# M4THYOU/TokenDagger

Hardware: AMD Instinct MI355X
Metric: GB/s raw text tokenized (Llama-4 vocab, 1024 MB corpus) (higher is better)
Workload: dtype u8; 1 GPU; Llama-4-Scout vocab, 1024 MiB synthetic english text, 1741775 documents, CoreBPE::encode semantics, input resident in HBM; bytes=1073741824, docs=1741775, bytes_rank0=1073741824, docs_rank0=1741775, parallelism=single GPU

## Files before the change

### tokendagger_amd/csrc/td_common.h

```cpp
#pragma once
#include <stdint.h>

#include "../../include/tokendagger_hip.h"

#if defined(__HIP__)
#define TD_HD __host__ __device__ inline __attribute__((always_inline))
#else
#define TD_HD inline
#endif

namespace td {

enum : uint32_t {
    C_OTHER = 0,
    C_APOS = 1,
    C_SLASH = 2,
    C_SP = 3,
    C_WS = 4,
    C_CRLF = 5,
    C_UP = 6,
    C_LW = 7,
    C_LB = 8,
    C_MK = 9,
    C_NUM = 10,
// ... 501 lines not shown
    MK_COUNT
};
struct BitWin {
    uint64_t m[MK_COUNT];
};

TD_HD int td_ctz64(uint64_t x) {
#if defined(__HIP_DEVICE_COMPILE__)
    return x ? (int)__builtin_ctzll(x) : 64;
#else
    return x ? (int)__builtin_ctzll(x) : 64;
#endif
}
TD_HD int td_top64(uint64_t x) { return 64 - (int)__builtin_clzll(x); }
TD_HD int td_run_end(uint64_t m, int f) { return f >= 64 ? 64 : f + td_ctz64(~(m >> f)); }
TD_HD uint64_t td_bits_below(int n) { return n >= 64 ? ~0ull : ((1ull << n) - 1ull); }

TD_HD uint32_t mask_bits_of(uint32_t vp, uint32_t v, uint32_t pv = 0) {
    const uint32_t c = v & CLS_MASK;
    uint32_t r = 0;
    r |= in_set(M_U, c) ? (1u << MK_U) : 0u;
    r |= in_set(M_W, c) ? (1u << MK_W) : 0u;
    r |= in_set(M_X, c) ? (1u << MK_X) : 0u;
    r |= in_set(M_S, c) ? (1u << MK_S) : 0u;
    r |= (c == C_NUM) ? (1u << MK_N) : 0u;
    r |= (c == C_CRLF) ? (1u << MK_CR) : 0u;
    r |= in_set(M_TRAIL, c) ? (1u << MK_TR) : 0u;
    r |= (v & F_CONT) ? (1u << MK_C) : 0u;
    r |= (v & F_DOC) ? (1u << MK_D) : 0u;
    r |= (c == C_APOS) ? (1u << MK_A) : 0u;
    r |= (c == C_SP) ? (1u << MK_SP) : 0u;
    r |= is_sync(vp, v, pv) ? (1u << MK_SYNC) : 0u;
    return r;
}
struct WinP {
    const BitWin& w;
    int o, lim;
    uint64_t E;
    TD_HD WinP(const BitWin& w_, int o_, int avail) : w(w_), o(o_), lim(avail), E(w_.m[MK_D] & ~td_bits_below(o_ + 1)) {}
    TD_HD bool bit(int k, int i) const { return (w.m[k] >> i) & 1ull; }
    TD_HD bool ebit(int i) const { return (E >> i) & 1ull; }
    TD_HD int run_end(int k, int from) const { return td_run_end(w.m[k] & ~E, from); }
    TD_HD int run_end2(int k1, int k2, int from) const { return td_run_end((w.m[k1] | w.m[k2]) & ~E, from); }
    TD_HD int last_and(int k1, int k2, int lo, int hi) const {
        const uint64_t m = w.m[k1] & w.m[k2] & td_bits_below(hi) & ~td_bits_below(lo);
        return m ? td_top64(m) - 1 : -1;
    }
    TD_HD int last_set(int k, int lo, int hi) const {
        const uint64_t m = w.m[k] & td_bits_below(hi) & ~td_bits_below(lo);
        return m ? td_top64(m) - 1 : -1;
    }
    TD_HD int last_clear(int k, int lo, int hi) const {
        const uint64_t m = ~w.m[k] & td_bits_below(hi) & ~td_bits_below(lo);
        return m ? td_top64(m) - 1 : -1;
    }
};

struct BitWin32 {
    uint32_t m[MK_COUNT];
};
TD_HD int td_ctz32(uint32_t x) { return x ? (int)__builtin_ctz(x) : 32; }
struct WinP32 {
    const BitWin32& w;
    int o, lim;
    uint32_t E;
    TD_HD WinP32(const BitWin32& w_, int avail) : w(w_), o(0), lim(avail), E(w_.m[MK_D] & ~1u) {}
    TD_HD bool bit(int k, int i) const { return (w.m[k] >> i) & 1u; }
    TD_HD bool ebit(int i) const { return (E >> i) & 1u; }
    TD_HD int run_end(int k, int from) const { return from >= 32 ? 32 : from + td_ctz32(~((w.m[k] & ~E) >> from)); }
    TD_HD int run_end2(int k1, int k2, int from) const {
        return from >= 32 ? 32 : from + td_ctz32(~(((w.m[k1] | w.m[k2]) & ~E) >> from));
    }
    TD_HD static uint32_t below(int n) { return n >= 32 ? ~0u : ((1u << n) - 1u); }
    TD_HD int last_and(int k1, int k2, int lo, int hi) const {
        const uint32_t m = w.m[k1] & w.m[k2] & below(hi) & ~below(lo);
        return m ? 31 - (int)__builtin_clz(m) : -1;
    }
    TD_HD int last_set(int k, int lo, int hi) const {
        const uint32_t m = w.m[k] & below(hi) & ~below(lo);
        return m ? 31 - (int)__builtin_clz(m) : -1;
    }
    TD_HD int last_clear(int k, int lo, int hi) const {
        const uint32_t m = ~w.m[k] & below(hi) & ~below(lo);
        return m ? 31 - (int)__builtin_clz(m) : -1;
    }
};

template <class B>
TD_HD int scan_piece_fast32(const BitWin32& v, int avail, const B& bytes, uint32_t pv) {
    if (pv & (PV_GPT2 | PV_LEADING_CONTRACTION | PV_PLAIN_LETTERS | PV_WS_EOS_FIRST)) return -1;
    const uint32_t U = v.m[MK_U], W = v.m[MK_W], X = v.m[MK_X], S = v.m[MK_S], N = v.m[MK_N], CR = v.m[MK_CR], TR = v.m[MK_TR];
    const uint32_t C = v.m[MK_C], A = v.m[MK_A], SP = v.m[MK_SP];
    const uint32_t E = v.m[MK_D] & ~1u;
    const uint32_t lim = avail >= 32 ? 0u : ~0u << avail;
    const uint32_t Ue = U & ~E, We = W & ~E, Xe = X & ~E, Se = S & ~E, TRe = TR & ~E;
    const int p1 = 1 + td_ctz32(~(C >> 1));
    const bool u0 = U & 1u, w0 = W & 1u, x0 = X & 1u, s0 = S & 1u, n0 = N & 1u, cr0 = CR & 1u;
    bool bad = p1 >= avail || p1 > 4;
    const int p1c = p1 > 31 ? 31 : p1;
    const bool l0 = u0 || w0;
    const bool l1 = (x0 || s0) && !((E >> p1c) & 1u) && (((U | W) >> p1c) & 1u);
    const bool letters = !cr0 && !n0 && (l0 || l1);
    bad = bad || (letters && l0 && l1);
    const int st = l1 ? p1c : 0;
    const int q = st + td_ctz32(~(Ue >> st));
    const int qc = q > 31 ? 31 : q;
    const bool wf = ((We >> qc) & 1u) && q < 32;
    const int ew = wf ? qc + td_ctz32(~(We >> qc)) : q;
    const uint32_t uw = U & W & ((qc == 0 ? 0u : (~0u >> (32 - qc)))) & (~0u << st);
    const int e1 = wf ? ew : (uw ? 32 - (int)__builtin_clz(uw) : 0);
    const int el = e1 ? e1 : (q > st ? ew : 0);
    int e_let = el;
    if (!(pv & PV_NO_CONTRACTION)) {
        const int ec = el > 29 ? 29 : el;
        const bool apo = ((A >> ec) & 1u) && !((v.m[MK_D] >> ec) & 1u) && !((v.m[MK_D] >> (ec + 1)) & 1u);
        if (letters && el > 0 && apo) {
            if (el + 3 > avail) bad = true;
            else {
                const uint32_t b1 = bytes(el + 1), b2 = bytes(el + 2);
                const bool d2 = (v.m[MK_D] >> (ec + 2)) & 1u;
                const uint32_t c1 = b1 | 0x20u, c2 = b2 | 0x20u;
                if (b1 < 0x80u && (c1 == 's' || c1 == 't' || c1 == 'm' || c1 == 'd')) e_let = el + 2;
                else if (b1 < 0x80u && !d2 && b2 < 0x80u && ((c1 == 'r' && c2 == 'e') || (c1 == 'v' && c2 == 'e') || (c1 == 'l' && c2 == 'l'))) e_let = el + 3;
                else if (b1 == 0xC5u && !d2 && b2 == 0xBFu) e_let = el + 3;
            }
        }
    }
    bad = bad || (letters && (el == 0 || q >= avail || ew >= avail || el + 3 > avail));
    const int nmax = (pv & PV_SINGLE_DIGIT) ? 1 : 3;
    const int nrun = td_ctz32(~(N & ~E) | (1u << nmax));
    const int e_num = nrun < 1 ? 1 : nrun;
    bad = bad || (n0 && ((C & 0xEu) || e_num + 1 > avail));
    const bool psp = (SP & 1u) && ((X >> 1) & 1u) && !((E >> 1) & 1u);
    const bool punct = psp || x0;
    const int pst = psp ? 1 : 0;
    const int px = pst + td_ctz32(~(Xe >> pst));
    const int pxc = px > 31 ? 31 : px;
    const int e_p = px >= 32 ? 32 : pxc + td_ctz32(~(TRe >> pxc));
    bad = bad || (!letters && !n0 && punct && (px >= avail || e_p >= avail));
    const int sq = td_ctz32(~Se);
    const uint32_t below = sq >= 32 ? ~0u : ((1u << sq) - 1u);
    const uint32_t crs = CR & below;
    const uint32_t leads = ~C & below & ~1u;
    const int e_s = crs ? 32 - (int)__builtin_clz(crs)
                        : (sq < 32 && ((E >> sq) & 1u)) ? sq
                        : leads ? 31 - (int)__builtin_clz(leads) : sq;
    bad = bad || (!letters && !n0 && !punct && s0 && sq >= avail);
    (void)lim;
    const int e = letters ? e_let : n0 ? e_num : punct ? e_p : s0 ? e_s : p1;
    return (bad || e <= 0 || e > avail) ? -1 : e;
}

TD_HD uint64_t td_land(uint64_t M, uint64_t A) { return ((M + (A & M)) & ~M) | (A & ~M); }
TD_HD uint64_t td_brev64(uint64_t x) {
#if defined(__clang__)
    return __builtin_bitreverse64(x);
#else
    x = ((x >> 1) & 0x5555555555555555ull) | ((x & 0x5555555555555555ull) << 1);
    x = ((x >> 2) & 0x3333333333333333ull) | ((x & 0x3333333333333333ull) << 2);
    x = ((x >> 4) & 0x0F0F0F0F0F0F0F0Full) | ((x & 0x0F0F0F0F0F0F0F0Full) << 4);
    return __builtin_bswap64(x);
#endif
}
constexpr uint32_t PV_WORD_RULES_OK = PV_NO_CONTRACTION | PV_SINGLE_DIGIT;
TD_HD uint64_t split_unresolved_heads(const BitWin& w, uint32_t pv, uint64_t* extra = nullptr) {
    const uint64_t SY = w.m[MK_SYNC];
    if (extra) *extra = 0;
    if (pv & ~PV_WORD_RULES_OK) return SY;
    const uint64_t nD = ~w.m[MK_D];
    const uint64_t U = w.m[MK_U] & nD, W = w.m[MK_W] & nD, X = w.m[MK_X] & nD, S = w.m[MK_S] & nD, N = w.m[MK_N] & nD;
    const uint64_t CR = w.m[MK_CR] & nD, TR = w.m[MK_TR] & nD, C = w.m[MK_C] & nD, SP = w.m[MK_SP] & nD;
    const uint64_t H = SY & nD;
    const uint64_t L = U | W, Up = U & ~W, Xn = X & ~L;
    const uint64_t pfx = H & (X | S) & ~CR & ~L;
    const uint64_t p1 = td_land(C, pfx << 1);
    const uint64_t a1 = (H & L) | (p1 & L);
    uint64_t good = td_land(W, td_land(Up, a1));
    const uint64_t hn = H & N;
    const uint64_t near = (pv & PV_SINGLE_DIGIT) ? (hn << 1) : ((hn << 1) | (hn << 2) | (hn << 3));
    const uint64_t ln = td_land(N, hn);
    good |= ln & near;
    if (extra && hn && !(pv & PV_SINGLE_DIGIT)) {
        const uint64_t NC = N & ~C;
        const uint64_t e3 = (hn << 3) & NC & (NC << 1) & (NC << 2);
        good |= ln & ((e3 << 1) | (e3 << 2) | (e3 << 3));
        *extra = e3;
    }
    const uint64_t b1 = (H & Xn) | ((H & SP & (Xn >> 1)) << 1);
    good |= td_land(TR, td_land(Xn, b1));
    const uint64_t hs = H & S;
    good |= td_land(S, hs) & ((CR << 1) | (hs << 1));
    const uint64_t bad_end = SY & ~good;
    const uint64_t zr = td_brev64(~SY);
    const uint64_t start = (td_brev64(bad_end) << 1) | 1ull;
    return td_brev64(td_land(zr, start));
}

struct ArrMaskP {
    const uint64_t* arr;
    int o, lim;
    TD_HD ArrMaskP(const uint64_t* a, int o_, int lim_) : arr(a), o(o_), lim(lim_) {}
    TD_HD uint64_t word(int k, int wi) const { return arr[wi * MK_COUNT + k]; }
    TD_HD uint64_t eword(int wi) const {
        const int wo = o >> 6;
        if (wi < wo) return 0;
        const uint64_t d = word(MK_D, wi);
        return wi == wo ? d & ~td_bits_below((o & 63) + 1) : d;
    }
    TD_HD bool bit(int k, int i) const { return (word(k, i >> 6) >> (i & 63)) & 1ull; }
    TD_HD bool ebit(int i) const { return i > o && bit(MK_D, i); }
    TD_HD int run_end(int k, int from) const {
        int i = from;
        while (i < lim) {
            const int wi = i >> 6, sh = i & 63;
            const uint64_t m = (word(k, wi) & ~eword(wi)) >> sh;
            const int t = td_ctz64(~m);
            if (t < 64 - sh) return i + t;
            i += 64 - sh;
        }
        return i;
    }
    TD_HD int run_end2(int k1, int k2, int from) const {
        int i = from;
        while (i < lim) {
            const int wi = i >> 6, sh = i & 63;
            const uint64_t m = ((word(k1, wi) | word(k2, wi)) & ~eword(wi)) >> sh;
            const int t = td_ctz64(~m);
            if (t < 64 - sh) return i + t;
            i += 64 - sh;
        }
        return i;
    }
    template <class F>
    TD_HD int last_where(const F& f, int lo, int hi) const {
        if (hi <= lo) return -1;
        for (int wi = (hi - 1) >> 6; wi >= (lo >> 6); --wi) {
            uint64_t m = f(wi);
            const int base = wi << 6;
            if (hi - base < 64) m &= td_bits_below(hi - base);
            if (lo > base) m &= ~td_bits_below(lo - base);
            if (m) return base + td_top64(m) - 1;
        }
        return -1;
    }
    TD_HD int last_and(int k1, int k2, int lo, int hi) const {
        return last_where([&](int wi) { return word(k1, wi) & word(k2, wi); }, lo, hi);
    }
    TD_HD int last_set(int k, int lo, int hi) const {
        return last_where([&](int wi) { return word(k, wi); }, lo, hi);
    }
    TD_HD int last_clear(int k, int lo, int hi) const {
        return last_where([&](int wi) { return ~word(k, wi); }, lo, hi);
    }
};

enum : int { CM_U = 0, CM_W, CM_X, CM_S, CM_NRAW, CM_CR, CM_TR, CM_C, CM_SYNC, CM_COUNT };
template <class V, class W>
TD_HD void cm_expand(V& v, const W* s, W d) {
    v.m[MK_U] = s[CM_U]; v.m[MK_W] = s[CM_W]; v.m[MK_X] = s[CM_X]; v.m[MK_S] = s[CM_S];
    v.m[MK_N] = s[CM_NRAW] & ~(s[CM_X] | s[CM_S]);
    v.m[MK_CR] = s[CM_CR]; v.m[MK_TR] = s[CM_TR]; v.m[MK_C] = s[CM_C];
    v.m[MK_D] = d;
    v.m[MK_A] = s[CM_NRAW] & s[CM_X];
    v.m[MK_SP] = s[CM_NRAW] & s[CM_S];
    v.m[MK_SYNC] = s[CM_SYNC];
}
struct CompactMaskP {
    const uint32_t* arr;
    const uint32_t* doc;
    int stride;
    int o, lim;
    TD_HD CompactMaskP(const uint32_t* a, int stride_, const uint32_t* d, int o_, int lim_) : arr(a), doc(d), stride(stride_), o(o_), lim(lim_) {}
    TD_HD uint64_t stored(int s, int wi) const { return ((uint64_t)arr[s * stride + 2 * wi + 1] << 32) | arr[s * stride + 2 * wi]; }
    TD_HD uint64_t dword64(int wi) const { return ((uint64_t)doc[2 * wi + 1] << 32) | doc[2 * wi]; }
    TD_HD uint64_t word(int k, int wi) const {
        switch (k) {
            case MK_U: return stored(CM_U, wi);
            case MK_W: return stored(CM_W, wi);
            case MK_X: return stored(CM_X, wi);
            case MK_S: return stored(CM_S, wi);
            case MK_N: return stored(CM_NRAW, wi) & ~(stored(CM_X, wi) | stored(CM_S, wi));
            case MK_CR: return stored(CM_CR, wi);
            case MK_TR: return stored(CM_TR, wi);
            case MK_C: return stored(CM_C, wi);
            case MK_D: return dword64(wi);
            case MK_A: return stored(CM_NRAW, wi) & stored(CM_X, wi);
            case MK_SP: return stored(CM_NRAW, wi) & stored(CM_S, wi);
            default: return stored(CM_SYNC, wi);
        }
    }
    TD_HD uint64_t eword(int wi) const {
        const int wo = o >> 6;
        if (wi < wo) return 0;
        const uint64_t d = dword64(wi);
        return wi == wo ? d & ~td_bits_below((o & 63) + 1) : d;
    }
    TD_HD bool bit(int k, int i) const { return (word(k, i >> 6) >> (i & 63)) & 1ull; }
    TD_HD bool ebit(int i) const { return i > o && bit(MK_D, i); }
    template <class F>
    TD_HD int run_where(const F& f, int from) const {
        int i = from;
        while (i < lim) {
            const int wi = i >> 6, sh = i & 63;
            const uint64_t m = (f(wi) & ~eword(wi)) >> sh;
            const int t = td_ctz64(~m);
            if (t < 64 - sh) return i + t;
            i += 64 - sh;
        }
        return i;
    }
    TD_HD int run_end(int k, int from) const { return run_where([&](int wi) { return word(k, wi); }, from); }
    TD_HD int run_end2(int k1, int k2, int from) const { return run_where([&](int wi) { return word(k1, wi) | word(k2, wi); }, from); }
    template <class F>
    TD_HD int last_where(const F& f, int lo, int hi) const {
        if (hi <= lo) return -1;
        for (int wi = (hi - 1) >> 6; wi >= (lo >> 6); --wi) {
            uint64_t m = f(wi);
            const int base = wi << 6;
            if (hi - base < 64) m &= td_bits_below(hi - base);
            if (lo > base) m &= ~td_bits_below(lo - base);
            if (m) return base + td_top64(m) - 1;
        }
        return -1;
    }
    TD_HD int last_and(int k1, int k2, int lo, int hi) const { return last_where([&](int wi) { return word(k1, wi) & word(k2, wi); }, lo, hi); }
    TD_HD int last_set(int k, int lo, int hi) const { return last_where([&](int wi) { return word(k, wi); }, lo, hi); }
    TD_HD int last_clear(int k, int lo, int hi) const { return last_where([&](int wi) { return ~word(k, wi); }, lo, hi); }
};

template <class P, class B>
TD_HD int scan_contraction_p(const P& p, const B& bytes, int e, bool leading = false) {
    if (e + 3 > p.lim) return -1;
    if (!p.bit(MK_A, e) || (p.bit(MK_D, e) && !leading)) return e;
    if (p.bit(MK_D, e + 1)) return e;
    const uint32_t b1 = bytes(e + 1);
    const bool d2 = p.bit(MK_D, e + 2);
    if (b1 < 0x80) {
        const uint32_t l1 = b1 | 0x20;
        if (l1 == 's' || l1 == 't' || l1 == 'm' || l1 == 'd') return e + 2;
        if (d2) return e;
        const uint32_t b2 = bytes(e + 2);
        if (b2 < 0x80) {
            const uint32_t l2 = b2 | 0x20;
            if ((l1 == 'r' && l2 == 'e') || (l1 == 'v' && l2 == 'e') || (l1 == 'l' && l2 == 'l')) return e + 3;
// ... 322 lines not shown
```

### tokendagger_amd/csrc/td_kernels.hip

```cpp
#include <hip/hip_runtime.h>
#include <stdlib.h>

#include "td_kernels.h"

namespace td {

#ifdef TD_ABLATE
#define TD_STOP(n) (a.stop_after == (n))
#else
#define TD_STOP(n) false
#endif

struct LdsSrc {
    const uint8_t* txt;
    const uint32_t* docw;
    int64_t lo, hi;
    __device__ __forceinline__ uint32_t byte(int64_t i) const { return txt[i]; }
    __device__ __forceinline__ bool doc(int64_t i) const { return (docw[i >> 5] >> (i & 31)) & 1u; }
};
struct GlobSrc {
    const uint8_t* text;
    const uint32_t* docbits;
    int64_t lo, hi;
    __device__ __forceinline__ uint32_t byte(int64_t i) const { return text[i]; }
// ... 1026 lines not shown
                auto bytes_below = [](int nb) { return nb >= 8 ? ~0ull : ((1ull << (8 * nb)) - 1ull); };
                {
                    const int lc0 = td_ctz64(~ct & HB) >> 3, lcd = (int)td_ctz32(docb | 0x100u);
                    lead_conts = lc0 < lcd ? lc0 : lcd;
                }
                uint32_t kj[4], ndj[4], cpj[4], uj[4];
                bool tbj[4];
#pragma unroll
                for (int j = 0; j < 4; ++j) {
                    const bool have = ld != 0;
                    const int k = have ? td_ctz64(ld) >> 3 : 0;
                    ld &= ld - 1ull;
#ifndef TD_DECODE_BRANCHY
                    const uint32_t dlo = k < 4 ? t8.x : t8.y, dhi = k < 4 ? t8.y : t8n.x;
                    const uint32_t x = __funnelshift_r(dlo, dhi, 8u * ((uint32_t)k & 3u));
                    const uint32_t b = x & 0xFFu;
                    const uint32_t need = utf8_declared_len(b) - 1u;
                    const int pos = pos0 + k;
                    const uint32_t cm = (0xC0C0C000u >> (8u * (3u - need))) & 0xC0C0C000u;
                    const bool ok = have & (need > 0) & (pos + (int)need < (int)src.hi) & (pos >= (int)src.lo) & (((docb >> (k + 1)) & ((1u << need) - 1u)) == 0u) &
                                    ((x & cm) == (cm & 0x80808000u));
                    const uint32_t c1 = (x >> 8) & 0x3Fu, c2 = (x >> 16) & 0x3Fu, c3 = (x >> 24) & 0x3Fu;
                    uint32_t c = ((b & (0x3Fu >> need)) << 6) | c1;
                    c = need >= 2u ? (c << 6) | c2 : c;
                    c = need >= 3u ? (c << 6) | c3 : c;
#else
                    const uint64_t hi8 = ((uint64_t)t8n.y << 32) | t8n.x;
                    const uint64_t w = (lo8 >> (8 * k)) | ((hi8 << 8) << (56 - 8 * k));
                    const uint32_t b = (uint32_t)w & 0xFFu, c1 = (uint32_t)(w >> 8) & 0xFFu, c2 = (uint32_t)(w >> 16) & 0xFFu, c3 = (uint32_t)(w >> 24) & 0xFFu;
                    const uint32_t need = utf8_declared_len(b) - 1u;
                    const int pos = pos0 + k;
                    const bool ok = have && need > 0 && pos + (int)need < (int)src.hi && pos >= (int)src.lo && !((docb >> (k + 1)) & ((1u << need) - 1u)) &&
                                    (c1 & 0xC0) == 0x80 && (need < 2 || (c2 & 0xC0) == 0x80) && (need < 3 || (c3 & 0xC0) == 0x80);
                    const uint32_t c = (need == 1) ? ((b & 0x1F) << 6) | (c1 & 0x3F)
                                     : (need == 2) ? ((b & 0x0F) << 12) | ((c1 & 0x3F) << 6) | (c2 & 0x3F)
                                                   : ((b & 0x07) << 18) | ((c1 & 0x3F) << 12) | ((c2 & 0x3F) << 6) | (c3 & 0x3F);
#endif
                    tbj[j] = ok && c <= 0x10FFFFu && !(c >= 0xD800u && c <= 0xDFFFu);
                    cpj[j] = tbj[j] ? c : 0u;
                    kj[j] = (uint32_t)k;
                    ndj[j] = ok ? need : 0u;
                    uj[j] = t_u1[cpj[j] >> 8];
                }
#pragma unroll
                for (int j = 0; j < 4; ++j) uj[j] = t_u2[uj[j] * 256u + (cpj[j] & 255u)];
                uint64_t cov = 0;
                int remaining = 0, last_lead = -1;
#pragma unroll
                for (int j = 0; j < 4; ++j) {
                    if (ndj[j]) {
                        const uint32_t f = tbj[j] ? (uint32_t)s_fcls[uj[j] & 15u] : (uint32_t)FB_X;
                        const uint32_t bm = ndj[j] == 3u ? 0xFFFFFFFFu : ((1u << (8u * (ndj[j] + 1u))) - 1u);
                        const uint32_t pat = ((f * 0x01010101u) | 0x80808000u) & bm;
                        const int sh = 8 * (int)kj[j];
                        F = (F & ~((uint64_t)bm << sh)) | ((uint64_t)pat << sh);
                        cov |= (uint64_t)(bm & 0x80808080u) << sh;
                        last_lead = (int)kj[j];
                        remaining = ((int)kj[j] + (int)ndj[j] > 7) ? (int)kj[j] + (int)ndj[j] - 7 : 0;
                    }
                }
                const uint64_t lcm = bytes_below(lead_conts);
                for (uint64_t gen = na & ~cov & ~lcm; gen; gen &= gen - 1ull) {
                    const int k = td_ctz64(gen) >> 3;
                    const uint32_t f = feature_at_v(t_ascii, t_u1, t_u2, s_txt, s_doc, (int)src.lo, (int)src.hi, pos0 + k);
                    F = (F & ~(0xFFull << (8 * k))) | ((uint64_t)f << (8 * k));
                }
                F &= ~lcm;
                flo = (uint32_t)F;
                fhi = (uint32_t)(F >> 32);
                const uint64_t starts = HB & ~(cov & ct) & ~lcm;
                if (starts) {
                    const int last = (63 - (int)__builtin_clzll(starts)) >> 3;
                    st_out = ((uint32_t)(F >> (8 * last)) & 0x7Fu) | ((uint32_t)(last == last_lead ? remaining : 0) << 9);
                } else {
                    st_out = 0x100u;
                }
            }
            {
                uint32_t st_in = __shfl_up(st_out, 1);
                if (lane == 0) st_in = carry_st;
                carry_st = (uint32_t)__builtin_amdgcn_readlane((int)st_out, 63);
                if (lead_conts) {
                    const bool known = !(st_in & 0x100u);
                    const int claim = (int)(st_in >> 9);
                    for (int k = 0; k < lead_conts; ++k) {
                        const uint32_t f = (known && k < claim) ? ((st_in & 0xFFu) | FB_C) : feature_at_v(t_ascii, t_u1, t_u2, s_txt, s_doc, (int)src.lo, (int)src.hi, it * 8 + k);
                        if (k < 4) flo |= f << (8 * k); else fhi |= f << (8 * (k - 4));
                    }
                }
            }
            uint32_t pf = __shfl_up(fhi >> 24, 1);
            if (lane == 0 && q > 0) pf = carry_pf;
            carry_pf = (uint32_t)__builtin_amdgcn_readlane((int)(fhi >> 24), 63);
            if (lane == 0 && q == 0) {
                pf = 0;
                if (it > 0) {
                    const uint32_t pb = s_txt[it * 8 - 1];
                    pf = (pb < 0x80) ? (uint32_t)s_lut[pb] : feature_at_v(t_ascii, t_u1, t_u2, s_txt, s_doc, (int)src.lo, (int)src.hi, it * 8 - 1);
                }
            }
            emit_masks(it, flo, fhi, pf);
        }
        }
        __syncthreads();
        FZ_TICK(1)
        if (tid == 0) s_nonascii = 0;
        if (TD_STOP(12)) continue;

        {
            constexpr bool FAST = !(PV & (PV_GPT2 | PV_LEADING_CONTRACTION | PV_PLAIN_LETTERS | PV_WS_EOS_FIRST));
            auto load_view64 = [&](BitWin& v, int j) {
                uint64_t s[CM_COUNT];
#pragma unroll
                for (int k = 0; k < CM_COUNT; ++k) s[k] = ((uint64_t)s_cm[k * CM_STRIDE + j + 1] << 32) | s_cm[k * CM_STRIDE + j];
                cm_expand(v, s, ((uint64_t)s_doc[j + 1] << 32) | s_doc[j]);
            };
            auto load_view32 = [&](BitWin32& v, int j, uint32_t sh) {
                uint32_t s[CM_COUNT];
#pragma unroll
                for (int k = 0; k < CM_COUNT; ++k) s[k] = __funnelshift_r(s_cm[k * CM_STRIDE + j], s_cm[k * CM_STRIDE + j + 1], sh);
                cm_expand(v, s, __funnelshift_r(s_doc[j], s_doc[j + 1], sh));
            };
            auto defer = [&](int64_t g) {
                if (FUSED) s_defer = 1;
                const uint32_t q = atomicAdd(a->slow_count, 1u);
                if (q < a->slow_cap) a->slow_list[q] = g;
                else raise(a, TD_E_SCRATCH, g);
            };
            auto mark = [&](int q) { atomicOr(&s_start[q >> 5], 1u << (q & 31)); };
            auto sync_at = [&](int q) { return (s_cm[CM_SYNC * CM_STRIDE + (q >> 5)] >> (q & 31)) & 1u; };
            auto crossed = [&](int e) {
                if (FUSED) s_cross = e;
                if (tile + 1 < a->n_stiles) a->tile_carry[tile + 1] = wg0 + e;
            };
            auto walk = [&](int p) {
                for (;;) {
                    const int e = scan_piece_lds<PV>(s_cm, s_doc, s_txt, p);
                    if (e < 0) { if (p >= K_HL) defer(wg0 + p); return; }
                    if (e >= tile_hi) { crossed(e); return; }
                    if (sync_at(e)) return;
                    if (e >= K_HL) mark(e);
                    p = e;
                }
            };
            const int b0 = K_HL + tid * 32;
            uint32_t mine = 0;
            uint32_t extra_hi = 0;
            {
                BitWin wv;
                load_view64(wv, b0 >> 5);
                uint32_t sy = (uint32_t)wv.m[MK_SYNC];
                const int room = tile_hi - b0;
                if (room < 32) sy = room <= 0 ? 0u : sy & ((1u << room) - 1u);
                uint32_t st0 = sy, un;
                if (wv.m[MK_N] != 0ull) {
                    uint64_t extra = 0;
                    un = (uint32_t)split_unresolved_heads(wv, PV, &extra) & sy;
                    extra &= (uint64_t)sy << 3;
                    extra &= room >= 64 ? ~0ull : room <= 0 ? 0ull : ((1ull << room) - 1ull);
                    st0 |= (uint32_t)extra;
                    extra_hi = (uint32_t)(extra >> 32);
                } else {
                    un = (uint32_t)split_unresolved_heads(wv, PV) & sy;
                }
                s_start[b0 >> 5] = st0;
                if (sy) atomicMax(&s_last, b0 + 31 - (int)__clz(sy));
                const uint32_t cnt = __popc(un);
                const uint32_t incl = wave_incl_scan(cnt, lane);
                uint32_t base = 0;
                if (lane == 63 && incl) base = atomicAdd(&s_nh, incl);
                base = (uint32_t)__builtin_amdgcn_readlane((int)base, 63);
                uint32_t idx = base + incl - cnt;
                while (un) {
                    const int bit = __ffs(un) - 1;
                    un &= un - 1u;
                    if (idx < (uint32_t)KS_HCAP) s_heads[idx] = (uint16_t)(b0 + bit); else mine |= 1u << bit;
                    ++idx;
                }
            }
            __syncthreads();
            FZ_TICK(2)
            if (extra_hi) atomicOr(&s_start[(b0 >> 5) + 1], extra_hi);
            if (TD_STOP(13)) continue;
            {
                const uint32_t nh = s_nh < (uint32_t)KS_HCAP ? s_nh : (uint32_t)KS_HCAP;
                int p = -1;
                if (tid == 0) {
                    static_assert(K_HL % 64 == 0 && K_HL >= 64, "left halo = whole mask words");
                    const uint32_t* const sync32 = s_cm + CM_SYNC * CM_STRIDE;
                    if (!(sync32[K_HL / 32] & 1u)) {
                        int sp = -1;
                        for (int w = K_HL / 64 - 1; w >= 0 && sp < 0; --w) {
                            uint64_t m = ((uint64_t)sync32[2 * w + 1] << 32) | sync32[2 * w];
                            if (w == 0) m &= ~0xFull;
                            if (m) sp = w * 64 + td_top64(m) - 1;
                        }
                        if (sp < 0) { a->tile_flag[tile] = 1; atomicAdd(a->far_count, 1u); if (FUSED) s_defer = 1; }
                        else p = sp;
                    }
                }
                if (tid == 1 && s_last >= 0) p = s_last;
                bool more = true;
                for (;;) {
                    const uint64_t nb = __ballot(p < 0);
                    if (nb && more) {
                        uint32_t base = 0;
                        if (lane == __ffsll((unsigned long long)nb) - 1) base = atomicAdd(&s_cur, (uint32_t)__popcll(nb));
                        base = (uint32_t)__builtin_amdgcn_readlane((int)base, __ffsll((unsigned long long)nb) - 1);
                        more = base + (uint32_t)__popcll(nb) < nh;
                        if (p < 0) {
                            const uint32_t idx = base + __builtin_amdgcn_mbcnt_hi((uint32_t)(nb >> 32), __builtin_amdgcn_mbcnt_lo((uint32_t)nb, 0u));
                            if (idx < nh) p = s_heads[idx];
                        }
                    }
                    if (!__ballot(p >= 0)) break;
                    if (p >= 0) {
                        BitWin32 v;
                        load_view32(v, p >> 5, (uint32_t)(p & 31));
                        const int avail = (K_LIM - p < 32) ? (K_LIM - p) : 32;
                        auto bytes = [&](int q) { return (uint32_t)s_txt[p + q]; };
                        const int r = FAST ? scan_piece_fast32(v, avail, bytes, PV) : scan_piece_p(WinP32(v, avail), bytes, PV);
                        if (r < 0) {
                            const uint32_t ci = atomicAdd(&s_ncold, 1u);
                            if (ci < (uint32_t)KS_CCAP) s_cold[ci] = (uint16_t)p; else walk(p);
                            p = -1;
                        } else {
                            const int e = p + r;
                            bool stop = true;
                            if (e >= tile_hi) crossed(e);
                            else {
                                stop = (r < 32) ? ((v.m[MK_SYNC] >> r) & 1u) : sync_at(e);
                                if (!stop && e >= K_HL) mark(e);
                            }
                            p = stop ? -1 : e;
                        }
                    }
                }
            }
            __syncthreads();
            {
                const uint32_t nc = s_ncold < (uint32_t)KS_CCAP ? s_ncold : (uint32_t)KS_CCAP;
                for (uint32_t i = tid; i < nc; i += K_THREADS) walk(s_cold[i]);
                while (mine) {
                    const int bit = __ffs(mine) - 1;
                    mine &= mine - 1u;
                    walk(b0 + bit);
                }
            }
        }
        __syncthreads();
        FZ_TICK(3)
        if (tid < KS_TILE / 32) {
            const int64_t g = tile_g0 + (int64_t)tid * 32;
            if (g < a->n) {
                uint32_t v = s_start[K_HL / 32 + tid];
                if (g + 32 > a->n) v &= (1u << (int)(a->n - g)) - 1u;
                TD_NT_STORE(v, &a->startbits[(tile_g0 >> 5) + tid]);
            }
        }
        if constexpr (DRAW) {
            if constexpr (!DIRECT) {
                next_tile = __builtin_amdgcn_readfirstlane(s_next[par]);
                if (tid == 0) s_next[par ^ 1] = (int)(2u * gridDim.x + atomicAdd(a->tile_draw, 1u));
                par = __builtin_amdgcn_readfirstlane(par ^ 1);
            } else {
                next_tile = __builtin_amdgcn_readfirstlane(s_next[0]);
            }
            if (next_tile < a->n_stiles) load_window((int64_t)next_tile * KS_TILE - K_HL);
        } else if (FUSED && tile + (int)gridDim.x < a->n_stiles) {
            load_window(wg0 + (int64_t)gridDim.x * KS_TILE);
        }
        }
        if constexpr (FUSED) {
            constexpr int NT4 = KS_TILE / K_TILE;
            static_assert(NT4 == 2 && KS_CHUNK == 32, "two token tiles, a 32-bit START word per lane");
            const int cross = s_cross;
            const bool tile_deferred = s_defer != 0 || cross < 0;
            uint16_t* const s_plist = reinterpret_cast<uint16_t*>(s_R + FZ_R_PLIST);
            uint16_t* const s_coldk = reinterpret_cast<uint16_t*>(s_R + FZ_R_COLDK);
            uint16_t* const s_pb = reinterpret_cast<uint16_t*>(s_R + FZ_R_PB);
            const int wv = tid >> 6;
            const int tile4 = tile * NT4;
            const bool two = K_HL + K_TILE < tile_hi;
            const int b0 = K_HL + tid * KS_CHUNK;
            const uint32_t smask0 = s_start[b0 >> 5];
            const uint32_t cnt = __popc(smask0);
            const uint32_t incl = wave_incl_scan(cnt, lane);
            if (lane == 63) s_wave[wv] = incl;
            if (tid == 0) { s_hflags[0] = 0; s_hflags[1] = 0; s_nrec[0] = 0; s_nrec[1] = 0; s_ncoldp = 0; }
            __syncthreads();
            const uint32_t w0s = s_wave[0], w1s = s_wave[1], w2s = s_wave[2], w3s = s_wave[3];
            const uint32_t np = w0s + w1s + w2s + w3s, n0 = w0s + w1s;
            const uint32_t pbase = (wv > 0 ? w0s : 0u) + (wv > 1 ? w1s : 0u) + (wv > 2 ? w2s : 0u) + incl - cnt;
            const bool cand = DIRECT && !s_brk;
            auto break_chain = [&]() {
                __hip_atomic_store(&a->tile_state[tile], TS_BROKEN << 62, __ATOMIC_RELAXED, __HIP_MEMORY_SCOPE_AGENT);
                s_brk = 1u;
            };
            if (tile_deferred || np > (uint32_t)FZ_NPC) {
                if (tid == 0) {
                    const uint32_t at = atomicAdd(a->deferred_count, two ? 2u : 1u);
                    a->deferred_list[at] = (uint32_t)tile4;
                    if (two) a->deferred_list[at + 1] = (uint32_t)tile4 + 1u;
                    if (DIRECT) break_chain();
                }
            } else {
                {
                    uint32_t k = pbase, m = smask0;
                    while (m) {
                        const int b = __ffs(m) - 1;
                        m &= m - 1;
                        s_plist[k++] = (uint16_t)(b0 + b);
                    }
                }
                s_pb[tid] = (uint16_t)pbase;
                if (tid == 0) s_plist[np] = (uint16_t)cross;
                const uint64_t fdd = fd0 != 0xFFFFFFFFu ? fd0 : fd1;
                if (cand && tid == 0) { s_pd[ring][PD_FDD] = (uint32_t)fdd; s_pd[ring][PD_TILE] = (uint32_t)tile; s_pd[ring][PD_NP] = np; s_pd[ring][PD_N0] = n0; }
                const int64_t dmine = (int64_t)fdd + tid;
                const int64_t dpos = (fdd != 0xFFFFFFFFu && dmine < a->n_docs) ? a->doc_offsets[dmine] : a->n;
                __syncthreads();
                FZ_TICK(4)
                uint32_t* const slab = a->slab + ((size_t)blockIdx.x * SLAB_RING + ring) * SLAB_WORDS;
                uint32_t* const dst0 = cand ? slab : a->stage + (size_t)tile4 * K_STAGE;
                uint32_t* const dst1 = cand ? slab : dst0 + K_STAGE - n0;
                auto note_miss = [&](uint32_t k, uint32_t res) {
                    const uint32_t h = k >= n0 ? 1u : 0u;
                    const uint32_t mi = atomicAdd(&s_nrec[h], 1u);
                    if (mi < (uint32_t)K_MISS_LISTED_MAX) s_rec[h][mi] = ((k - (h ? n0 : 0u)) << 19) | (res & 0x7FFFFu);
                };
                auto miss_marker = [&](int i, uint32_t len) { return TOK_MISS | ((uint32_t)((i - K_HL) & (K_TILE - 1)) << 7) | len; };
                typedef uint32_t u32x4 __attribute__((ext_vector_type(4)));
                typedef const u32x4 __attribute__((address_space(1)))* gslot_t;
                gslot_t const p12 = (gslot_t)(uintptr_t)T->piece12_slots;
                const uint32_t p12_mask = T->piece12_mask;
                const bool fastpath = a->use_fastpath != 0;
                for (uint32_t kb = tid; kb < np; kb += K_THREADS * FZ_PB) {
                    u32x4 sl[FZ_PB];
                    uint32_t kk0[FZ_PB], kk1[FZ_PB], kk2[FZ_PB], il[FZ_PB];
#pragma unroll
                    for (int q = 0; q < FZ_PB; ++q) {
                        const uint32_t k = kb + (uint32_t)q * K_THREADS;
                        const bool on = k < np;
                        const int i = on ? s_plist[k] : K_HL;
                        const uint32_t len = on ? (uint32_t)s_plist[k + 1] - (uint32_t)i : 0u;
                        const uint32_t* wp = reinterpret_cast<const uint32_t*>(s_txt) + (i >> 2);
                        const uint32_t sh = (i & 3) * 8;
                        const uint32_t w0 = wp[0], w1 = wp[1], w2 = wp[2], w3 = wp[3];
                        const uint4 km = reinterpret_cast<const uint4*>(s_kmask)[len < P12_MAXLEN ? len : P12_MAXLEN];
                        kk0[q] = __funnelshift_r(w0, w1, sh) & km.x;
                        kk1[q] = __funnelshift_r(w1, w2, sh) & km.y;
                        kk2[q] = __funnelshift_r(w2, w3, sh) & km.z;
                        il[q] = ((uint32_t)i << 16) | (len < 0xFFFFu ? len : 0xFFFFu);
                        if (on) sl[q] = p12[hash_piece12(kk0[q], kk1[q], kk2[q], len) & p12_mask];
                    }
#pragma unroll
                    for (int q = 0; q < FZ_PB; ++q) {
                        const uint32_t k = kb + (uint32_t)q * K_THREADS;
                        if (k < np) {
                            const int i = (int)(il[q] >> 16);
                            const uint32_t len = il[q] & 0xFFFFu;
                            const u32x4 e = sl[q];
                            if (len <= P12_MAXLEN && fastpath &&
                                (e.w == 0u || (e.x == kk0[q] && e.y == kk1[q] && e.z == kk2[q] && (e.w >> 24) == (0x80u | len)))) {
                                const bool miss = e.w == 0u;
                                const uint32_t res = miss ? miss_marker(i, len) : (e.w & 0x1FFFFFu);
                                if (miss) {
                                    if (len == 1) raise(a, TD_E_UNKNOWN_BYTE, wg0 + i);
                                    note_miss(k, res);
                                }
                                (k < n0 ? dst0 : dst1)[k] = res;
                            } else {
                                const uint32_t j = atomicAdd(&s_ncoldp, 1u);
                                if (j < (uint32_t)FZ_CCAP) s_coldk[j] = (uint16_t)k;
                            }
                        }
                    }
                }
                __syncthreads();
                FZ_TICK(5)
                const uint32_t ncold = s_ncoldp;
                const bool cold_overflow = ncold > (uint32_t)FZ_CCAP;
                if (!cold_overflow) {
                    for (uint32_t c = tid; c < ncold; c += K_THREADS) {
                        const uint32_t k = s_coldk[c];
                        const int i = s_plist[k];
                        const uint32_t len = (uint32_t)s_plist[k + 1] - (uint32_t)i;
                        const uint32_t h = k >= n0 ? 1u : 0u;
                        uint32_t res = probe_piece_cold<true>(a, T, s_txt, T->byte_id, &s_hflags[h], wg0, i, len);
                        if ((res & 0xC0000000u) == TOK_MISS) { res = miss_marker(i, len); note_miss(k, res); }
                        (h ? dst1 : dst0)[k] = res;
                    }
                }
                __syncthreads();
                FZ_TICK(6)
                const bool resolved = cand && !cold_overflow && !(s_hflags[0] | s_hflags[1]) && s_nrec[0] <= (uint32_t)K_MISS_LISTED_MAX &&
                                      s_nrec[1] <= (uint32_t)K_MISS_LISTED_MAX;
                if (cold_overflow) {
                    if (tid == 0) {
                        const uint32_t at = atomicAdd(a->deferred_count, two ? 2u : 1u);
// ... 3729 lines not shown
```

Baseline: 487.7 GB/s.

## Resolve more pretokenizer split heads in bitmask phase, skip serial walk when none remain

Extends split_unresolved_heads so that heads at document boundaries, digit runs, whitespace line starts and ASCII/long-s contractions (read from LDS bytes) count as resolved without a scalar walk. The tile kernel now resolves the left-halo lead piece and the tile-end crossing from the bitmask, packing the crossing point into s_last. It skips the head-walking loop entirely when there are no unresolved heads and no lead. The aim is to cut the serial per-head piece scanning that dominates the split phase. In exchange it adds more bit logic per word, a per-lane byte loop for apostrophes, and extra risk of split mismatches at edge cases.

```diff
diff --git a/tokendagger_amd/csrc/td_common.h b/tokendagger_amd/csrc/td_common.h
--- a/tokendagger_amd/csrc/td_common.h
+++ b/tokendagger_amd/csrc/td_common.h
@@ -677,6 +677,16 @@
 }
 
 TD_HD uint64_t td_land(uint64_t M, uint64_t A) { return ((M + (A & M)) & ~M) | (A & ~M); }
+struct TdNoBytes { TD_HD uint32_t operator()(int) const { return 0u; } };
+template <class B> struct td_has_bytes { static constexpr bool value = true; };
+template <> struct td_has_bytes<TdNoBytes> { static constexpr bool value = false; };
+TD_HD bool td_wave_any(bool x) {
+#if defined(__HIP_DEVICE_COMPILE__)
+    return __builtin_amdgcn_ballot_w64(x) != 0ull;
+#else
+    return x;
+#endif
+}
 TD_HD uint64_t td_brev64(uint64_t x) {
 #if defined(__clang__)
     return __builtin_bitreverse64(x);
@@ -688,22 +698,47 @@
 #endif
 }
 constexpr uint32_t PV_WORD_RULES_OK = PV_NO_CONTRACTION | PV_SINGLE_DIGIT;
-TD_HD uint64_t split_unresolved_heads(const BitWin& w, uint32_t pv, uint64_t* extra = nullptr) {
+template <class B = TdNoBytes>
+TD_HD uint64_t split_unresolved_heads(const BitWin& w, uint32_t pv, uint64_t* extra = nullptr, const B* bytes = nullptr, uint64_t* line_starts = nullptr) {
     const uint64_t SY = w.m[MK_SYNC];
     if (extra) *extra = 0;
+    if (line_starts) *line_starts = 0;
     if (pv & ~PV_WORD_RULES_OK) return SY;
-    const uint64_t nD = ~w.m[MK_D];
-    const uint64_t U = w.m[MK_U] & nD, W = w.m[MK_W] & nD, X = w.m[MK_X] & nD, S = w.m[MK_S] & nD, N = w.m[MK_N] & nD;
-    const uint64_t CR = w.m[MK_CR] & nD, TR = w.m[MK_TR] & nD, C = w.m[MK_C] & nD, SP = w.m[MK_SP] & nD;
-    const uint64_t H = SY & nD;
-    const uint64_t L = U | W, Up = U & ~W, Xn = X & ~L;
-    const uint64_t pfx = H & (X | S) & ~CR & ~L;
+    const uint64_t D = w.m[MK_D], nD = ~D;
+    const uint64_t Ur = w.m[MK_U], Wr = w.m[MK_W], Xr = w.m[MK_X], Sr = w.m[MK_S];
+    const uint64_t W = Wr & nD, S = Sr & nD, N = w.m[MK_N] & nD;
+    const uint64_t CR = w.m[MK_CR] & nD, TR = w.m[MK_TR] & nD, C = w.m[MK_C] & nD;
+    const uint64_t H = SY & nD, HD = SY & D;
+    const uint64_t Lr = Ur | Wr, L = Lr & nD, Upr = Ur & ~Wr, Up = Upr & nD, Xnr = Xr & ~Lr, Xn = Xnr & nD;
+    const uint64_t pfx = SY & (Xr | Sr) & ~w.m[MK_CR] & ~Lr;
     const uint64_t p1 = td_land(C, pfx << 1);
     const uint64_t a1 = (H & L) | (p1 & L);
-    uint64_t good = td_land(W, td_land(Up, a1));
-    const uint64_t hn = H & N;
-    const uint64_t near = (pv & PV_SINGLE_DIGIT) ? (hn << 1) : ((hn << 1) | (hn << 2) | (hn << 3));
-    const uint64_t ln = td_land(N, hn);
+    uint64_t ll = td_land(W, td_land(Up, a1 | ((HD & Upr) << 1)) | ((HD & Wr & ~Upr) << 1));
+    uint64_t good = ll;
+    if (td_has_bytes<B>::value && !(pv & PV_NO_CONTRACTION)) {
+        uint64_t ap = ll & w.m[MK_A] & nD & ~(D >> 1) & td_bits_below(62);
+        if (td_wave_any(ap != 0ull)) {
+            uint64_t lc = 0;
+            while (ap) {
+                const int e = td_ctz64(ap);
+                ap &= ap - 1ull;
+                const uint32_t b1 = (*bytes)(e + 1), c1 = b1 | 0x20u;
+                int len = 0;
+                if (b1 < 0x80u && (c1 == 's' || c1 == 't' || c1 == 'm' || c1 == 'd')) len = 2;
+                else if (!((D >> (e + 2)) & 1ull)) {
+                    const uint32_t b2 = (*bytes)(e + 2), c2 = b2 | 0x20u;
+                    if (b1 < 0x80u && b2 < 0x80u && ((c1 == 'r' && c2 == 'e') || (c1 == 'v' && c2 == 'e') || (c1 == 'l' && c2 == 'l'))) len = 3;
+                    else if (b1 == 0xC5u && b2 == 0xBFu) len = 3;
+                }
+                if (len) lc |= 1ull << (e + len);
+            }
+            good |= lc;
+            ll |= lc;
+        }
+    }
+    const uint64_t hn = H & N, hnd = (HD & w.m[MK_N]) << 1;
+    const uint64_t near = (pv & PV_SINGLE_DIGIT) ? ((hn << 1) | hnd) : ((hn << 1) | (hn << 2) | (hn << 3) | hnd | (hnd << 1) | (hnd << 2));
+    const uint64_t ln = td_land(N, hn | hnd);
     good |= ln & near;
     if (extra && hn && !(pv & PV_SINGLE_DIGIT)) {
         const uint64_t NC = N & ~C;
@@ -711,10 +746,12 @@
         good |= ln & ((e3 << 1) | (e3 << 2) | (e3 << 3));
         *extra = e3;
     }
-    const uint64_t b1 = (H & Xn) | ((H & SP & (Xn >> 1)) << 1);
+    const uint64_t b1 = (H & Xn) | ((SY & w.m[MK_SP] & (Xn >> 1)) << 1) | ((HD & Xnr) << 1);
     good |= td_land(TR, td_land(Xn, b1));
-    const uint64_t hs = H & S;
-    good |= td_land(S, hs) & ((CR << 1) | (hs << 1));
+    const uint64_t hs = H & S, hsd = (HD & Sr) << 1;
+    const uint64_t lcr = line_starts ? ll & CR : 0ull;
+    good |= td_land(S, hs | hsd | lcr) & ((CR << 1) | (hs << 1) | hsd);
+    if (line_starts) *line_starts = lcr;
     const uint64_t bad_end = SY & ~good;
     const uint64_t zr = td_brev64(~SY);
     const uint64_t start = (td_brev64(bad_end) << 1) | 1ull;
diff --git a/tokendagger_amd/csrc/td_kernels.hip b/tokendagger_amd/csrc/td_kernels.hip
--- a/tokendagger_amd/csrc/td_kernels.hip
+++ b/tokendagger_amd/csrc/td_kernels.hip
@@ -1202,19 +1202,20 @@
                 uint32_t sy = (uint32_t)wv.m[MK_SYNC];
                 const int room = tile_hi - b0;
                 if (room < 32) sy = room <= 0 ? 0u : sy & ((1u << room) - 1u);
-                uint32_t st0 = sy, un;
-                if (wv.m[MK_N] != 0ull) {
-                    uint64_t extra = 0;
-                    un = (uint32_t)split_unresolved_heads(wv, PV, &extra) & sy;
-                    extra &= (uint64_t)sy << 3;
-                    extra &= room >= 64 ? ~0ull : room <= 0 ? 0ull : ((1ull << room) - 1ull);
-                    st0 |= (uint32_t)extra;
-                    extra_hi = (uint32_t)(extra >> 32);
-                } else {
-                    un = (uint32_t)split_unresolved_heads(wv, PV) & sy;
-                }
-                s_start[b0 >> 5] = st0;
-                if (sy) atomicMax(&s_last, b0 + 31 - (int)__clz(sy));
+                const uint64_t in_tile = room >= 64 ? ~0ull : room <= 0 ? 0ull : ((1ull << room) - 1ull);
+                uint64_t extra = 0, line_starts = 0;
+                auto wbytes = [&](int q) { return (uint32_t)s_txt[b0 + q]; };
+                uint32_t un = (uint32_t)split_unresolved_heads(wv, PV, &extra, &wbytes, &line_starts) & sy;
+                extra |= line_starts;
+                if (sy) {
+                    const int top = 31 - (int)__clz(sy);
+                    const uint64_t behind = (wv.m[MK_SYNC] | extra) & ~in_tile;
+                    const int cr = (((un >> top) & 1u) || !behind) ? 0 : b0 + td_ctz64(behind);
+                    atomicMax(&s_last, ((b0 + top) << 16) | cr);
+                }
+                extra &= in_tile;
+                s_start[b0 >> 5] = sy | (uint32_t)extra;
+                extra_hi = (uint32_t)(extra >> 32);
                 const uint32_t cnt = __popc(un);
                 const uint32_t incl = wave_incl_scan(cnt, lane);
                 uint32_t base = 0;
@@ -1228,28 +1229,43 @@
                     ++idx;
                 }
             }
-            __syncthreads();
-            FZ_TICK(2)
-            if (extra_hi) atomicOr(&s_start[(b0 >> 5) + 1], extra_hi);
-            if (TD_STOP(13)) continue;
-            {
-                const uint32_t nh = s_nh < (uint32_t)KS_HCAP ? s_nh : (uint32_t)KS_HCAP;
-                int p = -1;
-                if (tid == 0) {
-                    static_assert(K_HL % 64 == 0 && K_HL >= 64, "left halo = whole mask words");
-                    const uint32_t* const sync32 = s_cm + CM_SYNC * CM_STRIDE;
-                    if (!(sync32[K_HL / 32] & 1u)) {
-                        int sp = -1;
+            if (tid == 0) {
+                int sp = -1;
+                static_assert(K_HL % 64 == 0 && K_HL >= 64, "left halo = whole mask words");
+                const uint32_t* const sync32 = s_cm + CM_SYNC * CM_STRIDE;
+                if (!(sync32[K_HL / 32] & 1u)) {
+                    if (sync32[K_HL / 32 - 1]) {
+                        BitWin wl;
+                        load_view64(wl, K_HL / 32 - 1);
+                        const int top = 31 - (int)__clz((uint32_t)wl.m[MK_SYNC]);
+                        uint64_t extra = 0, line_starts = 0;
+                        auto lbytes = [&](int q) { return (uint32_t)s_txt[K_HL - 32 + q]; };
+                        const uint64_t un = split_unresolved_heads(wl, PV, &extra, &lbytes, &line_starts);
+                        const int room = tile_hi - K_HL;
+                        const uint32_t close = (uint32_t)(wl.m[MK_SYNC] >> 32) & (room >= 32 ? ~0u : (1u << room) - 1u);
+                        if (((un >> top) & 1ull) || !close) sp = K_HL - 32 + top;
+                        else s_start[K_HL / 32] |= (uint32_t)((extra | line_starts) >> 32) & (close - 1u) & ~close;
+                    } else {
                         for (int w = K_HL / 64 - 1; w >= 0 && sp < 0; --w) {
                             uint64_t m = ((uint64_t)sync32[2 * w + 1] << 32) | sync32[2 * w];
                             if (w == 0) m &= ~0xFull;
                             if (m) sp = w * 64 + td_top64(m) - 1;
                         }
                         if (sp < 0) { a->tile_flag[tile] = 1; atomicAdd(a->far_count, 1u); if (FUSED) s_defer = 1; }
-                        else p = sp;
                     }
                 }
-                if (tid == 1 && s_last >= 0) p = s_last;
+                s_heads[KS_HCAP] = (uint16_t)sp;
+            }
+            __syncthreads();
+            FZ_TICK(2)
+            if (extra_hi) atomicOr(&s_start[(b0 >> 5) + 1], extra_hi);
+            if (tid == 1 && s_last >= 0 && (s_last & 0xFFFF)) crossed(s_last & 0xFFFF);
+            if (TD_STOP(13)) continue;
+            const uint32_t lead = s_heads[KS_HCAP];
+            if (__builtin_amdgcn_readfirstlane((int)(s_nh | (lead ^ 0xFFFFu))) != 0) {
+            {
+                const uint32_t nh = s_nh < (uint32_t)KS_HCAP ? s_nh : (uint32_t)KS_HCAP;
+                int p = (tid == 0 && lead != 0xFFFFu) ? (int)lead : -1;
                 bool more = true;
                 for (;;) {
                     const uint64_t nb = __ballot(p < 0);
@@ -1296,6 +1312,7 @@
                     mine &= mine - 1u;
                     walk(b0 + bit);
                 }
+            }
             }
         }
         __syncthreads();
```

Result: no change. 491.0 GB/s, median of 6 (+0.7%).
